# facebookresearch/omni3d

Hardware: NVIDIA H100
Metric: images/sec DLA34 Cube R-CNN train step (higher is better)
Workload: dtype bf16

## Files before the change

omni3d_b200/csrc/c3d_common.cu:

```cuda
#include <stdarg.h>
#include <string.h>
#include "c3d_common.cuh"

namespace c3d {
static thread_local char g_err[512] = "";
char* last_error_buf() { return g_err; }
int32_t set_error(int32_t code, const char* fmt, ...) {
  va_list ap; va_start(ap, fmt);
  vsnprintf(g_err, sizeof(g_err), fmt, ap);
  va_end(ap);
  return code;
}
}

extern "C" const char* c3d_last_error(void) { return c3d::last_error_buf(); }
extern "C" int32_t c3d_abi_version(void) { return 2; }
```

omni3d_b200/csrc/roi_align.cu:

```cuda
#include <cuda_bf16.h>
#include <stdlib.h>
#include "c3d_common.cuh"

namespace c3d {
using bf16 = __nv_bfloat16;

struct RoiLevels {
  const bf16* feat[5];
  float* grad[5];
  int H[5], W[5];
  float scale[5];
  int num_levels;
  int num_images;
};

struct Tap { int y0, y1, x0, x1; float w1, w2, w3, w4; bool valid; };

__device__ __forceinline__ Tap make_tap(float y, float x, int H, int W) {
  Tap t;
  t.valid = !(y < -1.0f || y > (float)H || x < -1.0f || x > (float)W);
  if (y <= 0.f) y = 0.f;
  if (x <= 0.f) x = 0.f;
  int yl = (int)y, xl = (int)x, yh, xh;
  if (yl >= H - 1) { yh = yl = H - 1; y = (float)yl; } else yh = yl + 1;
  if (xl >= W - 1) { xh = xl = W - 1; x = (float)xl; } else xh = xl + 1;
  float ly = y - yl, lx = x - xl, hy = 1.f - ly, hx = 1.f - lx;
  t.y0 = yl; t.y1 = yh; t.x0 = xl; t.x1 = xh;
  t.w1 = hy * hx; t.w2 = hy * lx; t.w3 = ly * hx; t.w4 = ly * lx;
  return t;
}

__device__ __forceinline__ void acc8(float (&a)[8], const bf16* p, float w) {
  uint4 u = __ldg(reinterpret_cast<const uint4*>(p));
  const __nv_bfloat162* h = reinterpret_cast<const __nv_bfloat162*>(&u);
#pragma unroll
  for (int i = 0; i < 4; ++i) { float2 f = __bfloat1622float2(h[i]); a[2 * i] += w * f.x; a[2 * i + 1] += w * f.y; }
}

__device__ __forceinline__ bool roi_sane(const float* roi, const RoiLevels& L) {
  const float fb = roi[0], fl = roi[1];
  return fb >= 0.f && (L.num_images <= 0 || fb < (float)L.num_images) && fl >= 0.f && fl < (float)L.num_levels &&
         isfinite(roi[2]) && isfinite(roi[3]) && isfinite(roi[4]) && isfinite(roi[5]);
}

__global__ void roi_align_kernel(RoiLevels L, const float* __restrict__ rois, int R, int C, int PH, int PW,
                                 bf16* __restrict__ out) {
  const int warps_per_block = blockDim.x >> 5;
  const int lane = threadIdx.x & 31;
  const long long nbins = (long long)R * PH * PW;
  for (long long bin = (long long)blockIdx.x * warps_per_block + (threadIdx.x >> 5); bin < nbins;
       bin += (long long)gridDim.x * warps_per_block) {
    const int pw = (int)(bin % PW), ph = (int)((bin / PW) % PH), r = (int)(bin / ((long long)PW * PH));
    const float* roi = rois + (size_t)r * 6;
    if (!roi_sane(roi, L)) {
      for (int c = lane * 8; c < C; c += 256) *reinterpret_cast<uint4*>(out + (size_t)bin * C + c) = make_uint4(0, 0, 0, 0);
      continue;
    }
    const int b = (int)roi[0], lvl = (int)roi[1];
    const float sc = L.scale[lvl];
    const int H = L.H[lvl], W = L.W[lvl];
    const float sw = roi[2] * sc - 0.5f, sh = roi[3] * sc - 0.5f;
    const float rw = roi[4] * sc - 0.5f - sw, rh = roi[5] * sc - 0.5f - sh;
    const float bh = rh / PH, bw = rw / PW;
    const int gh = (int)ceilf(rh / PH), gw = (int)ceilf(rw / PW);
    const float cnt = fmaxf((float)(gh * gw), 1.f);
    const bf16* base = L.feat[lvl] + (size_t)b * H * W * C;
    for (int c = lane * 8; c < C; c += 256) {
      float a[8];
#pragma unroll
      for (int k = 0; k < 8; ++k) a[k] = 0.f;
      for (int iy = 0; iy < gh; ++iy) {
        const float y = sh + ph * bh + (iy + 0.5f) * bh / (float)gh;
        for (int ix = 0; ix < gw; ++ix) {
          const float x = sw + pw * bw + (ix + 0.5f) * bw / (float)gw;
          Tap t = make_tap(y, x, H, W);
          if (!t.valid) continue;
          acc8(a, base + ((size_t)t.y0 * W + t.x0) * C + c, t.w1); acc8(a, base + ((size_t)t.y0 * W + t.x1) * C + c, t.w2);
          acc8(a, base + ((size_t)t.y1 * W + t.x0) * C + c, t.w3); acc8(a, base + ((size_t)t.y1 * W + t.x1) * C + c, t.w4);
        }
      }
      uint4 u;
      __nv_bfloat162* h = reinterpret_cast<__nv_bfloat162*>(&u);
#pragma unroll
      for (int i = 0; i < 4; ++i) h[i] = __floats2bfloat162_rn(a[2 * i] / cnt, a[2 * i + 1] / cnt);
      *reinterpret_cast<uint4*>(out + (size_t)bin * C + c) = u;
    }
  }
}

constexpr int kTile = 8, kTileC = 256, kListCap = 2048;
constexpr int kBwdSmem = kTile * kTile * kTileC * 4;

__global__ void __launch_bounds__(kTileC)
roi_align_bwd_kernel(RoiLevels L, const float* __restrict__ rois, int R, int C, int PH, int PW, const bf16* __restrict__ dout) {
  extern __shared__ float sacc[];
  __shared__ int slist[kListCap];
  __shared__ int s_wc[kTileC / 32];
  __shared__ int s_n, s_touch;
  const int tid = threadIdx.x, lane = tid & 31, wid = tid >> 5;
  const int b = blockIdx.y;
  int lvl = 0, band = blockIdx.x;
  while (lvl < L.num_levels - 1 && band >= (L.H[lvl] + kTile - 1) / kTile) { band -= (L.H[lvl] + kTile - 1) / kTile; ++lvl; }
  const int H = L.H[lvl], W = L.W[lvl];
  if (band * kTile >= H) return;
  const float sc = L.scale[lvl];
  const int ty0 = band * kTile, ty1 = min(H, ty0 + kTile) - 1;
  float* gmap = L.grad[lvl] + (size_t)b * H * W * C;
  for (int r0 = 0; r0 < R;) {
    if (tid == 0) s_n = 0;
    __syncthreads();
    int r = r0;
    while (r < R) {
      const int idx = r + tid;
      bool pred = false;
      if (idx < R) {
        const float* roi = rois + (size_t)idx * 6;
        if (roi_sane(roi, L) && (int)roi[0] == b && (int)roi[1] == lvl) {
          const float sh = roi[3] * sc - 0.5f, eh = roi[5] * sc - 0.5f;
          pred = (int)floorf(sh) - 1 <= ty1 && (int)floorf(eh) + 1 >= ty0;
        }
      }
      const unsigned bal = __ballot_sync(0xffffffffu, pred);
      if (lane == 0) s_wc[wid] = __popc(bal);
      __syncthreads();
      int before = 0, total = 0;
      for (int w = 0; w < kTileC / 32; ++w) { total += s_wc[w]; if (w < wid) before += s_wc[w]; }
      const int n0 = s_n;
      const bool fits = n0 + total <= kListCap;
      if (fits && pred) slist[n0 + before + __popc(bal & ((1u << lane) - 1u))] = idx;
      __syncthreads();
      if (!fits) break;
      if (tid == 0) s_n = n0 + total;
      __syncthreads();
      r += kTileC;
    }
    r0 = r;
    const int n = s_n;
    for (int tx0 = 0; tx0 < W; tx0 += kTile) {
      const int tx1 = min(W, tx0 + kTile) - 1;
      for (int cc = 0; cc < C; cc += kTileC) {
        const int c = cc + tid;
        const bool cin = c < C;
        for (int p = 0; p < kTile * kTile; ++p) sacc[p * kTileC + tid] = 0.f;
        if (tid == 0) s_touch = 0;
        __syncthreads();
        for (int li = 0; li < n; ++li) {
          const int ri = slist[li];
          const float* roi = rois + (size_t)ri * 6;
          const float sw = roi[2] * sc - 0.5f, sh = roi[3] * sc - 0.5f;
          const float rw = roi[4] * sc - 0.5f - sw, rh = roi[5] * sc - 0.5f - sh;
          if ((int)floorf(sw) - 1 > tx1 || (int)floorf(sw + rw) + 1 < tx0) continue;
          const float bh = rh / PH, bw = rw / PW;
          const int gh = (int)ceilf(rh / PH), gw = (int)ceilf(rw / PW);
          const float cnt = fmaxf((float)(gh * gw), 1.f);
          for (int ph = 0; ph < PH; ++ph) {
            if ((int)floorf(sh + ph * bh) - 1 > ty1 || (int)floorf(sh + (ph + 1) * bh) + 1 < ty0) continue;
            for (int pw = 0; pw < PW; ++pw) {
              if ((int)floorf(sw + pw * bw) - 1 > tx1 || (int)floorf(sw + (pw + 1) * bw) + 1 < tx0) continue;
              const float g = cin ? __bfloat162float(dout[(((size_t)ri * PH + ph) * PW + pw) * C + c]) / cnt : 0.f;
              for (int iy = 0; iy < gh; ++iy) {
                const float y = sh + ph * bh + (iy + 0.5f) * bh / (float)gh;
                for (int ix = 0; ix < gw; ++ix) {
                  const float x = sw + pw * bw + (ix + 0.5f) * bw / (float)gw;
                  const Tap t = make_tap(y, x, H, W);
                  if (!t.valid) continue;
                  const int ys[4] = {t.y0, t.y0, t.y1, t.y1}, xs[4] = {t.x0, t.x1, t.x0, t.x1};
                  const float ws[4] = {t.w1, t.w2, t.w3, t.w4};
#pragma unroll
                  for (int j = 0; j < 4; ++j)
                    if (ys[j] >= ty0 && ys[j] <= ty1 && xs[j] >= tx0 && xs[j] <= tx1) {
                      sacc[((ys[j] - ty0) * kTile + (xs[j] - tx0)) * kTileC + tid] += ws[j] * g;
                      if (tid == 0) s_touch = 1;
                    }
                }
              }
            }
          }
        }
        __syncthreads();
        if (s_touch && cin) {
          for (int p = 0; p < kTile * kTile; ++p) {
            const int py = ty0 + p / kTile, px = tx0 + p % kTile;
            if (py <= ty1 && px <= tx1) gmap[((size_t)py * W + px) * C + c] += sacc[p * kTileC + tid];
          }
        }
        __syncthreads();
      }
    }
  }
}

static int32_t run(bool bwd, const c3d_roi_levels* lv, const float* rois, int R, int C, int PH, int PW, void* out,
                   const void* dout, cudaStream_t st) {
  if (!lv || lv->num_levels < 1 || lv->num_levels > 5 || C % 8 != 0) return set_error(C3D_EINVAL, "roi_align: bad args");
  if (R == 0) return C3D_OK;
  RoiLevels L;
  L.num_levels = lv->num_levels;
  L.num_images = lv->num_images;
  for (int i = 0; i < 5; ++i) {
    L.feat[i] = (const bf16*)lv->feat[i]; L.grad[i] = (float*)lv->grad[i];
    L.H[i] = lv->H[i]; L.W[i] = lv->W[i]; L.scale[i] = lv->scale[i];
  }
  if (!bwd) {
    long long nbins = (long long)R * PH * PW;
    long long blocks = (nbins + 7) / 8;
    if (blocks > kNumSMs * 16) blocks = kNumSMs * 16;
    roi_align_kernel<<<(unsigned)blocks, 256, 0, st>>>(L, rois, R, C, PH, PW, (bf16*)out);
    return check_launch("roi_align");
  }
  if (L.num_images <= 0) return set_error(C3D_EINVAL, "roi_align bwd: num_images must be set");
  static bool attr = false;
  if (!attr) {
    cudaError_t e = cudaFuncSetAttribute(roi_align_bwd_kernel, cudaFuncAttributeMaxDynamicSharedMemorySize, kBwdSmem);
    if (e != cudaSuccess) return set_error(C3D_ECUDA, "roi_align bwd smem attr: %s", cudaGetErrorString(e));
    attr = true;
  }
  int bands = 0;
  for (int i = 0; i < L.num_levels; ++i) bands += (L.H[i] + kTile - 1) / kTile;
  roi_align_bwd_kernel<<<dim3((unsigned)bands, (unsigned)L.num_images), kTileC, kBwdSmem, st>>>(L, rois, R, C, PH, PW, (const bf16*)dout);
  return check_launch("roi_align bwd");
}
}

extern "C" int32_t c3d_roi_align_fwd(const c3d_roi_levels* levels, const float* rois, int32_t R, int32_t C,
                                     int32_t pooled_h, int32_t pooled_w, void* out, void* stream) {
  if (!rois && R > 0) return c3d::set_error(C3D_EINVAL, "roi_align: null rois");
  return c3d::run(false, levels, rois, R, C, pooled_h, pooled_w, out, nullptr, (cudaStream_t)stream);
}
extern "C" int32_t c3d_roi_align_bwd(const c3d_roi_levels* levels, const float* rois, int32_t R, int32_t C,
                                     int32_t pooled_h, int32_t pooled_w, const void* dout, void* stream) {
  if (!rois && R > 0) return c3d::set_error(C3D_EINVAL, "roi_align: null rois");
  return c3d::run(true, levels, rois, R, C, pooled_h, pooled_w, nullptr, dout, (cudaStream_t)stream);
}
```

omni3d_b200/kernels.py:

```python
import ctypes

import torch

from . import _lib
from ._lib import ptr, stream

vp, i32, f32 = ctypes.c_void_p, ctypes.c_int32, ctypes.c_float


def bn_finalize(stats, count, eps, momentum, running_mean, running_var):
    L = _lib.lib()
    rows, _, C = stats.shape
    mean = torch.empty(C, device=stats.device, dtype=torch.float32)
    rstd = torch.empty(C, device=stats.device, dtype=torch.float32)
    scratch = torch.empty(128 * 2 * C + 64, device=stats.device, dtype=torch.float64)
    _lib.check(L.c3d_bn_finalize(ptr(stats), rows, C, float(count), eps, momentum, ptr(running_mean), ptr(running_var),
                                 ptr(mean), ptr(rstd), ptr(scratch), stream()), launches=1)
    return mean, rstd


def bn_apply(y, mean, rstd, gamma, beta, residual=None, relu=True, out=None):
    L = _lib.lib()
    C = y.shape[-1]
    P = y.numel() // C
# ... 85 lines not shown

def preprocess_images(images, mean, std, size_divisibility=64, cpad=16):
    L = _lib.lib()
    Hm = max(im.shape[1] for im in images)
    Wm = max(im.shape[2] for im in images)
    d = size_divisibility
    Hp, Wp = (Hm + d - 1) // d * d, (Wm + d - 1) // d * d
    out = torch.empty((len(images), Hp, Wp, cpad), device=images[0].device, dtype=torch.bfloat16)
    m = (f32 * 3)(*[float(v) for v in mean])
    s = (f32 * 3)(*[float(v) for v in std])
    for im in images:
        assert im.dtype in (torch.float32, torch.uint8) and im.is_contiguous() and im.is_cuda

    def run(ims, dst):
        n = len(ims)
        ptrs = (vp * n)(*[im.data_ptr() for im in ims])
        hs = (i32 * n)(*[im.shape[1] for im in ims])
        ws = (i32 * n)(*[im.shape[2] for im in ims])
        _lib.check(L.c3d_preprocess_batch(ptrs, hs, ws, n, int(ims[0].dtype == torch.uint8), ptr(dst), Hp, Wp, cpad, m, s,
                                          stream()), launches=(n + 63) // 64)
    if all(im.dtype == images[0].dtype for im in images):
        run(images, out)
    else:
        for i, im in enumerate(images):
            run([im], out[i])
    return out


def _levels(feats, strides, grads=None):
    lv = _lib.RoiLevels()
    lv.num_levels = len(feats)
    lv.num_images = feats[0].shape[0]
    for i, f in enumerate(feats):
        lv.feat[i] = f.data_ptr()
        lv.grad[i] = grads[i].data_ptr() if grads is not None else None
        lv.H[i], lv.W[i] = f.shape[1], f.shape[2]
        lv.scale[i] = 1.0 / strides[i]
    return lv


def roi_align_fwd(feats, strides, rois, pooled=7):
    L = _lib.lib()
    C = feats[0].shape[-1]
    R = rois.shape[0]
    out = torch.empty((R, pooled, pooled, C), device=feats[0].device, dtype=torch.bfloat16)
    lv = _levels(feats, strides)
    _lib.check(L.c3d_roi_align_fwd(ctypes.byref(lv), ptr(rois), R, C, pooled, pooled, ptr(out), stream()))
    return out


def roi_align_bwd(feats, strides, rois, dout, pooled=7):
    L = _lib.lib()
    C = feats[0].shape[-1]
    grads = [torch.zeros(f.shape, device=f.device, dtype=torch.float32) for f in feats]
    lv = _levels(feats, strides, grads)
    _lib.check(L.c3d_roi_align_bwd(ctypes.byref(lv), ptr(rois), rois.shape[0], C, pooled, pooled, ptr(dout), stream()))
    return grads


def grad_finite(flat_grad, flag):
    L = _lib.lib()
    _lib.check(L.c3d_grad_finite(ptr(flat_grad), flat_grad.numel(), ptr(flag), stream()))


def sgd_momentum(p, g, mom, lr, momentum, weight_decay, grad_scale=1.0, skip_flag=None):
    L = _lib.lib()
    if torch.is_tensor(lr):
        _lib.check(L.c3d_sgd_momentum_dev(ptr(p), ptr(g), ptr(mom), p.numel(), ptr(lr), momentum, weight_decay, grad_scale,
                                          ptr(skip_flag), stream()))
    else:
        _lib.check(L.c3d_sgd_momentum(ptr(p), ptr(g), ptr(mom), p.numel(), lr, momentum, weight_decay, grad_scale,
                                      ptr(skip_flag), stream()))


_nms_ws = {}


def nms_batched(boxes, nvalid, iou_thresh, max_keep, cats=None, maxc=None, trick_max_numel=20000, ncat=0, max_per_cat=0):
    L = _lib.lib()
    B, n, _ = boxes.shape
    boxes = boxes.contiguous()
    need = L.c3d_nms_workspace_bytes(B, n)
    key = boxes.device.index
    ws = _nms_ws.get(key)
    if ws is None or ws.numel() < need:
        ws = torch.empty(need, dtype=torch.uint8, device=boxes.device)
        _nms_ws[key] = ws
    keep = torch.empty((B, max_keep), dtype=torch.int32, device=boxes.device)
    cnt = torch.empty((B,), dtype=torch.int32, device=boxes.device)
    if ncat > 0 and cats is not None:
        _lib.check(L.c3d_nms_batched_grouped(ptr(boxes), ptr(nvalid), ptr(cats), ptr(maxc), trick_max_numel, B, n, iou_thresh,
                                             max_keep, ncat, max_per_cat, ptr(keep), ptr(cnt), ptr(ws), ws.numel(), stream()),
                   launches=4)
        return keep, cnt
    _lib.check(L.c3d_nms_batched(ptr(boxes), ptr(nvalid), ptr(cats), ptr(maxc), trick_max_numel, B, n, iou_thresh,
                                 max_keep, ptr(keep), ptr(cnt), ptr(ws), ws.numel(), stream()), launches=2)
    return keep, cnt


def anchor_match(anchors, gt_boxes, gt_valid, gt_ign, fg_thresh):
    L = _lib.lib()
    A = anchors.shape[0]
    B, G, _ = gt_boxes.shape
    dev = anchors.device
    anchors, gt_boxes = anchors.contiguous().float(), gt_boxes.contiguous().float()
    v8, i8 = gt_valid.to(torch.uint8).contiguous(), gt_ign.to(torch.uint8).contiguous()
    idx = torch.empty((B, A), dtype=torch.int64, device=dev)
# ... 266 lines not shown
```

omni3d_b200/nnfunc.py:

```python
import weakref

import torch

from . import _lib
from . import conv as K
from . import kernels as Kx

_pack_cache = {}
_lin_cache = {}
_epoch = 0


def invalidate_packed():
    global _epoch
    _epoch += 1
    _pack_cache.clear()
    _lin_cache.clear()


def _cache_key(w):
    if not isinstance(w, torch.nn.Parameter):
        return None, None
    return id(w), (w.data_ptr(), w._version, _epoch, tuple(w.shape), tuple(w.stride()))

# ... 348 lines not shown
            return fn(None)
        dwb = wgrad(wb, lambda g: K.linear_wgrad(x, dzb, dw=g, chw=chw))
        dwc = wgrad(wc, lambda g: K.linear_wgrad_blocks(x, dzc, B, Fc, S, dw=g, chw=chw))
        return dx, dwb, gbb if rb else None, dwc, gbc if rc else None, None, None, None, None


class MaxPool2(torch.autograd.Function):
    @staticmethod
    def forward(ctx, x):
        ctx.sink = _sink_of(x)
        x = x.contiguous()
        ctx.save_for_backward(x)
        return Kx.maxpool2_fwd(x)

    @staticmethod
    def backward(ctx, dy):
        (x,) = ctx.saved_tensors
        sink = ctx.sink
        if sink is not None and sink.buf is not None and sink.buf.dtype == x.dtype:
            Kx.maxpool2_bwd(x, dy, into=sink.buf)
            return None
        return _deliver(sink, Kx.maxpool2_bwd(x, dy))


class MaxPool3s2(torch.autograd.Function):

    @staticmethod
    def forward(ctx, x):
        x = x.contiguous()
        ctx.save_for_backward(x)
        return Kx.maxpool3s2_fwd(x)

    @staticmethod
    def backward(ctx, dy):
        (x,) = ctx.saved_tensors
        return Kx.maxpool3s2_bwd(x, dy)


class ROIAlign(torch.autograd.Function):

    @staticmethod
    def forward(ctx, rois, strides, pooled, *feats):
        ctx.sinks = [_sink_of(f) for f in feats]
        feats = [f.contiguous() for f in feats]
        ctx.save_for_backward(rois, *feats)
        ctx.cfg = (strides, pooled)
        return Kx.roi_align_fwd(feats, strides, rois, pooled)

    @staticmethod
    def backward(ctx, dout):
        rois, *feats = ctx.saved_tensors
        strides, pooled = ctx.cfg
        grads = Kx.roi_align_bwd(feats, strides, rois, dout.contiguous(), pooled)
        return (None, None, None) + tuple(_deliver(s, g.to(torch.bfloat16)) for s, g in zip(ctx.sinks, grads))


class CubeLossRows(torch.autograd.Function):

    @staticmethod
    def forward(ctx, raw, aux):
        raw, aux = raw.contiguous().float(), aux.contiguous().float()
        ctx.save_for_backward(raw, aux)
        out = Kx.cube_loss_fwd(raw, aux)
        ctx.mark_non_differentiable()
        return out

    @staticmethod
    def backward(ctx, dout):
        raw, aux = ctx.saved_tensors
        return Kx.cube_loss_bwd(raw, aux, dout[:, :6].contiguous().float()), None


class RPNLossSums(torch.autograd.Function):

    @staticmethod
    def forward(ctx, logits, deltas, labels, matched_idx, gt_boxes, anchors, weights):
        logits, deltas = logits.contiguous().float(), deltas.contiguous().float()
        labels, matched_idx = labels.to(torch.int8).contiguous(), matched_idx.contiguous()
        gt_boxes, anchors = gt_boxes.contiguous().float(), anchors.contiguous().float()
        ctx.save_for_backward(logits, deltas, labels, matched_idx, gt_boxes, anchors)
        ctx.weights = tuple(weights)
        return Kx.rpn_loss_fwd(logits, deltas, labels, matched_idx, gt_boxes, anchors, weights)

    @staticmethod
    def backward(ctx, dacc):
        logits, deltas, labels, matched_idx, gt_boxes, anchors = ctx.saved_tensors
        dacc = dacc.contiguous().float()
        dl, dd = Kx.rpn_loss_bwd(logits, deltas, labels, matched_idx, gt_boxes, anchors, ctx.weights, dacc[0:1], dacc[1:2])
        return dl, dd, None, None, None, None, None


class BoxLoss(torch.autograd.Function):

    @staticmethod
    def forward(ctx, pred, classes, valid, boxes, gt_boxes, K, weights):
        pred = pred.contiguous().float()
        classes, valid = classes.contiguous().to(torch.int64), valid.contiguous().to(torch.uint8)
        boxes, gt_boxes = boxes.contiguous().float(), gt_boxes.contiguous().float()
        acc = Kx.box_loss_fwd(pred, classes, valid, boxes, gt_boxes, K, weights)
        ctx.save_for_backward(pred, classes, valid, boxes, gt_boxes, acc)
        ctx.cfg = (K, tuple(weights))
        nv, nfg = acc[2].clamp(min=1.0), acc[3].clamp(min=1.0)
        den = torch.stack([nv, nv, nv, nfg, nfg])
        return torch.cat([torch.cat([acc[0:2], acc[4:7]]) / den, acc[2:4]])

    @staticmethod
    def backward(ctx, g):
# ... 29 lines not shown
```

Baseline: 360.8.

## Restructure ROIAlign backward into per-tile blocks with pre-bucketed ROI lists and bf16 output

ROIAlign backward gets a small pre-pass kernel that buckets ROIs by (image, level) into a compact list. The main backward kernel then launches one block per 8x8 spatial tile instead of one per row band, and each block filters only its segment's ROIs. Each thread now handles two channels with float2 smem accumulators at half the thread count. The kernel writes bf16 gradients directly, removing the fp32 zero-fill, the read-modify-write accumulation and the separate fp32-to-bf16 cast. The cost is an extra launch plus async malloc/free per call, and tile-level ROI rescanning may duplicate filtering work.

Result: faster. 394.9 (median of 6 runs) (+9.4%).

```diff
diff --git a/omni3d_b200/csrc/c3d_common.cu b/omni3d_b200/csrc/c3d_common.cu
--- a/omni3d_b200/csrc/c3d_common.cu
+++ b/omni3d_b200/csrc/c3d_common.cu
@@ -14,4 +14,4 @@
 }
 
 extern "C" const char* c3d_last_error(void) { return c3d::last_error_buf(); }
-extern "C" int32_t c3d_abi_version(void) { return 2; }
+extern "C" int32_t c3d_abi_version(void) { return 3; }
diff --git a/omni3d_b200/csrc/roi_align.cu b/omni3d_b200/csrc/roi_align.cu
--- a/omni3d_b200/csrc/roi_align.cu
+++ b/omni3d_b200/csrc/roi_align.cu
@@ -7,7 +7,7 @@
 
 struct RoiLevels {
   const bf16* feat[5];
-  float* grad[5];
+  void* grad[5];
   int H[5], W[5];
   float scale[5];
   int num_levels;
@@ -88,120 +88,218 @@
   }
 }
 
-constexpr int kTile = 8, kTileC = 256, kListCap = 2048;
+constexpr int kTile = 8, kTileC = 256, kBwdThreads = kTileC / 2, kListCap = 2048;
 constexpr int kBwdSmem = kTile * kTile * kTileC * 4;
 
-__global__ void __launch_bounds__(kTileC)
-roi_align_bwd_kernel(RoiLevels L, const float* __restrict__ rois, int R, int C, int PH, int PW, const bf16* __restrict__ dout) {
-  extern __shared__ float sacc[];
+struct BwdScratch {
+  int* seg_off;
+  int* seg_n;
+  int* list;
+};
+
+__device__ __forceinline__ int roi_key(const float* roi, const RoiLevels& L) {
+  return roi_sane(roi, L) ? (int)roi[0] * L.num_levels + (int)roi[1] : -1;
+}
+
+__global__ void __launch_bounds__(256) roi_bwd_list_kernel(RoiLevels L, const float* __restrict__ rois, int R, BwdScratch S) {
+  __shared__ int s_wc[8];
+  const int seg = blockIdx.x, tid = threadIdx.x, lane = tid & 31, wid = tid >> 5;
+  int below = 0, n = 0;
+  for (int r0 = 0; r0 < R; r0 += 256) {
+    const int k = r0 + tid < R ? roi_key(rois + (size_t)(r0 + tid) * 6, L) : -1;
+    below += __syncthreads_count(k >= 0 && k < seg);
+    n += __syncthreads_count(k == seg);
+  }
+  int* list = S.list + below;
+  int pos = 0;
+  for (int r0 = 0; r0 < R && pos < n; r0 += 256) {
+    const bool pred = r0 + tid < R && roi_key(rois + (size_t)(r0 + tid) * 6, L) == seg;
+    const unsigned bal = __ballot_sync(0xffffffffu, pred);
+    if (lane == 0) s_wc[wid] = __popc(bal);
+    __syncthreads();
+    int before = 0, total = 0;
+    for (int w = 0; w < 8; ++w) { total += s_wc[w]; if (w < wid) before += s_wc[w]; }
+    if (pred) list[pos + before + __popc(bal & ((1u << lane) - 1u))] = r0 + tid;
+    pos += total;
+    __syncthreads();
+  }
+  if (tid == 0) { S.seg_off[seg] = below; S.seg_n[seg] = n; }
+}
+
+__device__ __forceinline__ void axis_tap(float v, int n, int& lo, int& hi, float& l) {
+  if (v <= 0.f) v = 0.f;
+  lo = (int)v;
+  if (lo >= n - 1) { hi = lo = n - 1; v = (float)lo; } else hi = lo + 1;
+  l = v - lo;
+}
+
+__global__ void __launch_bounds__(kBwdThreads, 3)
+roi_bwd_kernel(RoiLevels L, const float* __restrict__ rois, int R, int C, int PH, int PW, const bf16* __restrict__ dout,
+               BwdScratch S) {
+  extern __shared__ float2 sacc[];
   __shared__ int slist[kListCap];
-  __shared__ int s_wc[kTileC / 32];
-  __shared__ int s_n, s_touch;
+  __shared__ int s_wc[kBwdThreads / 32];
   const int tid = threadIdx.x, lane = tid & 31, wid = tid >> 5;
-  const int b = blockIdx.y;
-  int lvl = 0, band = blockIdx.x;
-  while (lvl < L.num_levels - 1 && band >= (L.H[lvl] + kTile - 1) / kTile) { band -= (L.H[lvl] + kTile - 1) / kTile; ++lvl; }
-  const int H = L.H[lvl], W = L.W[lvl];
-  if (band * kTile >= H) return;
+  int u = blockIdx.x, lvl = 0, per_image = 0;
+  for (int l = 0; l < L.num_levels; ++l) per_image += ((L.H[l] + kTile - 1) / kTile) * ((L.W[l] + kTile - 1) / kTile);
+  const int b = u / per_image;
+  u -= b * per_image;
+  while (u >= ((L.H[lvl] + kTile - 1) / kTile) * ((L.W[lvl] + kTile - 1) / kTile)) {
+    u -= ((L.H[lvl] + kTile - 1) / kTile) * ((L.W[lvl] + kTile - 1) / kTile);
+    ++lvl;
+  }
+  const int H = L.H[lvl], W = L.W[lvl], tiles_x = (W + kTile - 1) / kTile;
+  const int ty0 = (u / tiles_x) * kTile, tx0 = (u % tiles_x) * kTile;
+  const int ty1 = min(H, ty0 + kTile) - 1, tx1 = min(W, tx0 + kTile) - 1;
   const float sc = L.scale[lvl];
-  const int ty0 = band * kTile, ty1 = min(H, ty0 + kTile) - 1;
-  float* gmap = L.grad[lvl] + (size_t)b * H * W * C;
-  for (int r0 = 0; r0 < R;) {
-    if (tid == 0) s_n = 0;
-    __syncthreads();
-    int r = r0;
-    while (r < R) {
-      const int idx = r + tid;
-      bool pred = false;
-      if (idx < R) {
-        const float* roi = rois + (size_t)idx * 6;
-        if (roi_sane(roi, L) && (int)roi[0] == b && (int)roi[1] == lvl) {
-          const float sh = roi[3] * sc - 0.5f, eh = roi[5] * sc - 0.5f;
-          pred = (int)floorf(sh) - 1 <= ty1 && (int)floorf(eh) + 1 >= ty0;
+  const int seg = b * L.num_levels + lvl;
+  const int n = R > 0 ? S.seg_n[seg] : 0;
+  const int* seg_list = R > 0 ? S.list + S.seg_off[seg] : nullptr;
+  bf16* gmap = reinterpret_cast<bf16*>(L.grad[lvl]) + (size_t)b * H * W * C;
+  for (int cc = 0; cc < C; cc += kTileC) {
+    const int c = cc + 2 * tid;
+    const bool cin = c < C;
+    for (int p = 0; p < kTile * kTile; ++p) sacc[p * kBwdThreads + tid] = make_float2(0.f, 0.f);
+    for (int i0 = 0; i0 < n;) {
+      int m = 0, i = i0;
+      while (i < n) {
+        bool pred = false;
+        int ri = 0;
+        if (i + tid < n) {
+          ri = seg_list[i + tid];
+          const float* roi = rois + (size_t)ri * 6;
+          const float sw = roi[2] * sc - 0.5f, sh = roi[3] * sc - 0.5f, eh = roi[5] * sc - 0.5f;
+          const float rw = roi[4] * sc - 0.5f - sw;
+          pred = (int)floorf(sh) - 1 <= ty1 && (int)floorf(eh) + 1 >= ty0 &&
+                 !((int)floorf(sw) - 1 > tx1 || (int)floorf(sw + rw) + 1 < tx0);
         }
+        const unsigned bal = __ballot_sync(0xffffffffu, pred);
+        if (lane == 0) s_wc[wid] = __popc(bal);
+        __syncthreads();
+        int before = 0, total = 0;
+        for (int w = 0; w < kBwdThreads / 32; ++w) { total += s_wc[w]; if (w < wid) before += s_wc[w]; }
+        const bool fits = m + total <= kListCap;
+        if (fits && pred) slist[m + before + __popc(bal & ((1u << lane) - 1u))] = ri;
+        __syncthreads();
+        if (!fits) break;
+        m += total;
+        i += kBwdThreads;
       }
-      const unsigned bal = __ballot_sync(0xffffffffu, pred);
-      if (lane == 0) s_wc[wid] = __popc(bal);
-      __syncthreads();
-      int before = 0, total = 0;
-      for (int w = 0; w < kTileC / 32; ++w) { total += s_wc[w]; if (w < wid) before += s_wc[w]; }
-      const int n0 = s_n;
-      const bool fits = n0 + total <= kListCap;
-      if (fits && pred) slist[n0 + before + __popc(bal & ((1u << lane) - 1u))] = idx;
-      __syncthreads();
-      if (!fits) break;
-      if (tid == 0) s_n = n0 + total;
-      __syncthreads();
-      r += kTileC;
-    }
-    r0 = r;
-    const int n = s_n;
-    for (int tx0 = 0; tx0 < W; tx0 += kTile) {
-      const int tx1 = min(W, tx0 + kTile) - 1;
-      for (int cc = 0; cc < C; cc += kTileC) {
-        const int c = cc + tid;
-        const bool cin = c < C;
-        for (int p = 0; p < kTile * kTile; ++p) sacc[p * kTileC + tid] = 0.f;
-        if (tid == 0) s_touch = 0;
-        __syncthreads();
-        for (int li = 0; li < n; ++li) {
-          const int ri = slist[li];
-          const float* roi = rois + (size_t)ri * 6;
-          const float sw = roi[2] * sc - 0.5f, sh = roi[3] * sc - 0.5f;
-          const float rw = roi[4] * sc - 0.5f - sw, rh = roi[5] * sc - 0.5f - sh;
-          if ((int)floorf(sw) - 1 > tx1 || (int)floorf(sw + rw) + 1 < tx0) continue;
-          const float bh = rh / PH, bw = rw / PW;
-          const int gh = (int)ceilf(rh / PH), gw = (int)ceilf(rw / PW);
-          const float cnt = fmaxf((float)(gh * gw), 1.f);
-          for (int ph = 0; ph < PH; ++ph) {
-            if ((int)floorf(sh + ph * bh) - 1 > ty1 || (int)floorf(sh + (ph + 1) * bh) + 1 < ty0) continue;
-            for (int pw = 0; pw < PW; ++pw) {
-              if ((int)floorf(sw + pw * bw) - 1 > tx1 || (int)floorf(sw + (pw + 1) * bw) + 1 < tx0) continue;
-              const float g = cin ? __bfloat162float(dout[(((size_t)ri * PH + ph) * PW + pw) * C + c]) / cnt : 0.f;
-              for (int iy = 0; iy < gh; ++iy) {
-                const float y = sh + ph * bh + (iy + 0.5f) * bh / (float)gh;
-                for (int ix = 0; ix < gw; ++ix) {
-                  const float x = sw + pw * bw + (ix + 0.5f) * bw / (float)gw;
-                  const Tap t = make_tap(y, x, H, W);
-                  if (!t.valid) continue;
-                  const int ys[4] = {t.y0, t.y0, t.y1, t.y1}, xs[4] = {t.x0, t.x1, t.x0, t.x1};
-                  const float ws[4] = {t.w1, t.w2, t.w3, t.w4};
+      i0 = i;
+      for (int li = 0; li < m; ++li) {
+        const int ri = slist[li];
+        const float* roi = rois + (size_t)ri * 6;
+        const float sw = roi[2] * sc - 0.5f, sh = roi[3] * sc - 0.5f;
+        const float rw = roi[4] * sc - 0.5f - sw, rh = roi[5] * sc - 0.5f - sh;
+        const float bh = rh / PH, bw = rw / PW;
+        const int gh = (int)ceilf(rh / PH), gw = (int)ceilf(rw / PW);
+        const float cnt = fmaxf((float)(gh * gw), 1.f);
+        const bf16* dr = dout + (size_t)ri * PH * PW * C + c;
+        for (int ph = 0; ph < PH; ++ph) {
+          if ((int)floorf(sh + ph * bh) - 1 > ty1 || (int)floorf(sh + (ph + 1) * bh) + 1 < ty0) continue;
+          for (int pw = 0; pw < PW; ++pw) {
+            if ((int)floorf(sw + pw * bw) - 1 > tx1 || (int)floorf(sw + (pw + 1) * bw) + 1 < tx0) continue;
+            float2 g = make_float2(0.f, 0.f);
+            if (cin) {
+              g = __bfloat1622float2(*reinterpret_cast<const __nv_bfloat162*>(dr + (size_t)(ph * PW + pw) * C));
+              g.x = g.x / cnt; g.y = g.y / cnt;
+            }
+            for (int iy = 0; iy < gh; ++iy) {
+              const float y = sh + ph * bh + (iy + 0.5f) * bh / (float)gh;
+              if (y < -1.0f || y > (float)H) continue;
+              int y0, y1; float ly;
+              axis_tap(y, H, y0, y1, ly);
+              if (y1 < ty0 || y0 > ty1) continue;
+              const float hy = 1.f - ly;
+              for (int ix = 0; ix < gw; ++ix) {
+                const float x = sw + pw * bw + (ix + 0.5f) * bw / (float)gw;
+                if (x < -1.0f || x > (float)W) continue;
+                int x0, x1; float lx;
+                axis_tap(x, W, x0, x1, lx);
+                if (x1 < tx0 || x0 > tx1) continue;
+                const float hx = 1.f - lx;
+                const int ys[4] = {y0, y0, y1, y1}, xs[4] = {x0, x1, x0, x1};
+                const float ws[4] = {hy * hx, hy * lx, ly * hx, ly * lx};
 #pragma unroll
-                  for (int j = 0; j < 4; ++j)
-                    if (ys[j] >= ty0 && ys[j] <= ty1 && xs[j] >= tx0 && xs[j] <= tx1) {
-                      sacc[((ys[j] - ty0) * kTile + (xs[j] - tx0)) * kTileC + tid] += ws[j] * g;
-                      if (tid == 0) s_touch = 1;
-                    }
-                }
+                for (int j = 0; j < 4; ++j)
+                  if (ys[j] >= ty0 && ys[j] <= ty1 && xs[j] >= tx0 && xs[j] <= tx1) {
+                    float2* a = sacc + ((ys[j] - ty0) * kTile + (xs[j] - tx0)) * kBwdThreads + tid;
+                    float2 v = *a;
+                    v.x += ws[j] * g.x; v.y += ws[j] * g.y;
+                    *a = v;
+                  }
               }
             }
           }
         }
-        __syncthreads();
-        if (s_touch && cin) {
-          for (int p = 0; p < kTile * kTile; ++p) {
-            const int py = ty0 + p / kTile, px = tx0 + p % kTile;
-            if (py <= ty1 && px <= tx1) gmap[((size_t)py * W + px) * C + c] += sacc[p * kTileC + tid];
-          }
+      }
+      __syncthreads();
+    }
+    if (cin) {
+      for (int p = 0; p < kTile * kTile; ++p) {
+        const int y = ty0 + p / kTile, x = tx0 + p % kTile;
+        if (y <= ty1 && x <= tx1) {
+          const float2 v = sacc[p * kBwdThreads + tid];
+          *reinterpret_cast<__nv_bfloat162*>(gmap + ((size_t)y * W + x) * C + c) =
+              __floats2bfloat162_rn(0.f + v.x, 0.f + v.y);
         }
-        __syncthreads();
       }
     }
   }
+}
+
+static size_t align16(size_t n) { return (n + 15) & ~(size_t)15; }
+
+static int32_t run_bwd(const RoiLevels& L, const float* rois, int R, int C, int PH, int PW, const bf16* dout, cudaStream_t st) {
+  static bool attr = false;
+  if (!attr) {
+    cudaError_t e = cudaFuncSetAttribute(roi_bwd_kernel, cudaFuncAttributeMaxDynamicSharedMemorySize, kBwdSmem);
+    if (e != cudaSuccess) return set_error(C3D_ECUDA, "roi_align bwd smem attr: %s", cudaGetErrorString(e));
+    attr = true;
+  }
+  long long units = 0;
+  for (int i = 0; i < L.num_levels; ++i)
+    units += (long long)((L.H[i] + kTile - 1) / kTile) * ((L.W[i] + kTile - 1) / kTile);
+  units *= L.num_images;
+  if (units == 0) return C3D_OK;
+  if (units > 0x7fffffffLL) return set_error(C3D_EINVAL, "roi_align bwd: maps too large");
+  const int nseg = L.num_images * L.num_levels;
+  BwdScratch S{};
+  void* scratch = nullptr;
+  if (R > 0) {
+    const size_t seg_bytes = align16((size_t)nseg * 4);
+    cudaError_t e = cudaMallocAsync(&scratch, 2 * seg_bytes + (size_t)R * 4, st);
+    if (e != cudaSuccess) return set_error(C3D_ECUDA, "roi_align bwd scratch: %s", cudaGetErrorString(e));
+    char* p = static_cast<char*>(scratch);
+    S.seg_off = reinterpret_cast<int*>(p);
+    S.seg_n = reinterpret_cast<int*>(p + seg_bytes);
+    S.list = reinterpret_cast<int*>(p + 2 * seg_bytes);
+    roi_bwd_list_kernel<<<(unsigned)nseg, 256, 0, st>>>(L, rois, R, S);
+    int32_t rc = check_launch("roi_bwd_list_kernel");
+    if (rc != C3D_OK) { cudaFreeAsync(scratch, st); return rc; }
+  }
+  roi_bwd_kernel<<<(unsigned)units, kBwdThreads, kBwdSmem, st>>>(L, rois, R, C, PH, PW, dout, S);
+  int32_t rc = check_launch("roi_bwd_kernel");
+  if (scratch) {
+    cudaError_t e = cudaFreeAsync(scratch, st);
+    if (rc == C3D_OK && e != cudaSuccess) rc = set_error(C3D_ECUDA, "roi_align bwd scratch free: %s", cudaGetErrorString(e));
+  }
+  return rc;
 }
 
 static int32_t run(bool bwd, const c3d_roi_levels* lv, const float* rois, int R, int C, int PH, int PW, void* out,
                    const void* dout, cudaStream_t st) {
   if (!lv || lv->num_levels < 1 || lv->num_levels > 5 || C % 8 != 0) return set_error(C3D_EINVAL, "roi_align: bad args");
-  if (R == 0) return C3D_OK;
+  if (R < 0 || PH < 1 || PW < 1) return set_error(C3D_EINVAL, "roi_align: bad sizes");
   RoiLevels L;
   L.num_levels = lv->num_levels;
   L.num_images = lv->num_images;
   for (int i = 0; i < 5; ++i) {
-    L.feat[i] = (const bf16*)lv->feat[i]; L.grad[i] = (float*)lv->grad[i];
+    L.feat[i] = (const bf16*)lv->feat[i]; L.grad[i] = lv->grad[i];
     L.H[i] = lv->H[i]; L.W[i] = lv->W[i]; L.scale[i] = lv->scale[i];
   }
   if (!bwd) {
+    if (R == 0) return C3D_OK;
     long long nbins = (long long)R * PH * PW;
     long long blocks = (nbins + 7) / 8;
     if (blocks > kNumSMs * 16) blocks = kNumSMs * 16;
@@ -209,16 +307,9 @@
     return check_launch("roi_align");
   }
   if (L.num_images <= 0) return set_error(C3D_EINVAL, "roi_align bwd: num_images must be set");
-  static bool attr = false;
-  if (!attr) {
-    cudaError_t e = cudaFuncSetAttribute(roi_align_bwd_kernel, cudaFuncAttributeMaxDynamicSharedMemorySize, kBwdSmem);
-    if (e != cudaSuccess) return set_error(C3D_ECUDA, "roi_align bwd smem attr: %s", cudaGetErrorString(e));
-    attr = true;
-  }
-  int bands = 0;
-  for (int i = 0; i < L.num_levels; ++i) bands += (L.H[i] + kTile - 1) / kTile;
-  roi_align_bwd_kernel<<<dim3((unsigned)bands, (unsigned)L.num_images), kTileC, kBwdSmem, st>>>(L, rois, R, C, PH, PW, (const bf16*)dout);
-  return check_launch("roi_align bwd");
+  for (int i = 0; i < L.num_levels; ++i)
+    if (!L.grad[i] || L.H[i] < 1 || L.W[i] < 1) return set_error(C3D_EINVAL, "roi_align bwd: level %d needs a map", i);
+  return run_bwd(L, rois, R, C, PH, PW, (const bf16*)dout, st);
 }
 }
 
diff --git a/omni3d_b200/kernels.py b/omni3d_b200/kernels.py
--- a/omni3d_b200/kernels.py
+++ b/omni3d_b200/kernels.py
@@ -161,7 +161,7 @@
 def roi_align_bwd(feats, strides, rois, dout, pooled=7):
     L = _lib.lib()
     C = feats[0].shape[-1]
-    grads = [torch.zeros(f.shape, device=f.device, dtype=torch.float32) for f in feats]
+    grads = [torch.empty(f.shape, device=f.device, dtype=torch.bfloat16) for f in feats]
     lv = _levels(feats, strides, grads)
     _lib.check(L.c3d_roi_align_bwd(ctypes.byref(lv), ptr(rois), rois.shape[0], C, pooled, pooled, ptr(dout), stream()))
     return grads
diff --git a/omni3d_b200/nnfunc.py b/omni3d_b200/nnfunc.py
--- a/omni3d_b200/nnfunc.py
+++ b/omni3d_b200/nnfunc.py
@@ -424,7 +424,7 @@
         rois, *feats = ctx.saved_tensors
         strides, pooled = ctx.cfg
         grads = Kx.roi_align_bwd(feats, strides, rois, dout.contiguous(), pooled)
-        return (None, None, None) + tuple(_deliver(s, g.to(torch.bfloat16)) for s, g in zip(ctx.sinks, grads))
+        return (None, None, None) + tuple(_deliver(s, g) for s, g in zip(ctx.sinks, grads))
 
 
 class CubeLossRows(torch.autograd.Function):
```

## Bucket ROIs per image/level and rework RoIAlign backward into work-list scatter

Applied to the files above, without the earlier changes.

Adds a single-block bucketing kernel that sorts ROIs by (image, level) into offset/index lists. The backward tile kernel then reads only its own bucket instead of rescanning and filtering all ROIs in every band block. It also builds per-tile lists of active bins and samples, which spreads the per-sample tap work across all threads, and writes every tile in place of read-modify-write. That lets the Python side drop the zero-fill of the gradient buffers. The cost is a second launch, an async allocation on every call, a larger shared-memory footprint, and more barrier-heavy inner loops.

Result: faster. 392.6 before, 420.5 after, median of 6 (+7.1%).

```diff
diff --git a/omni3d_b200/csrc/c3d_common.cu b/omni3d_b200/csrc/c3d_common.cu
--- a/omni3d_b200/csrc/c3d_common.cu
+++ b/omni3d_b200/csrc/c3d_common.cu
@@ -14,4 +14,4 @@
 }
 
 extern "C" const char* c3d_last_error(void) { return c3d::last_error_buf(); }
-extern "C" int32_t c3d_abi_version(void) { return 2; }
+extern "C" int32_t c3d_abi_version(void) { return 3; }
diff --git a/omni3d_b200/csrc/roi_align.cu b/omni3d_b200/csrc/roi_align.cu
--- a/omni3d_b200/csrc/roi_align.cu
+++ b/omni3d_b200/csrc/roi_align.cu
@@ -14,6 +14,26 @@
   int num_images;
 };
 
+struct RoiGeom { float sw, sh, rw, rh, bw, bh, cnt; int gw, gh; };
+
+__device__ __forceinline__ RoiGeom roi_geom(const float* roi, float sc, int PH, int PW) {
+  RoiGeom g;
+  g.sw = fmaf(roi[2], sc, -0.5f);
+  g.sh = fmaf(roi[3], sc, -0.5f);
+  g.rw = __fsub_rn(fmaf(roi[4], sc, -0.5f), g.sw);
+  g.rh = __fsub_rn(fmaf(roi[5], sc, -0.5f), g.sh);
+  g.bw = __fdiv_rn(g.rw, (float)PW);
+  g.bh = __fdiv_rn(g.rh, (float)PH);
+  g.gw = (int)ceilf(g.bw);
+  g.gh = (int)ceilf(g.bh);
+  g.cnt = fmaxf((float)(g.gh * g.gw), 1.f);
+  return g;
+}
+
+__device__ __forceinline__ float sample_at(float s, int p, float b, int i, int n) {
+  return __fadd_rn(fmaf((float)p, b, s), __fdiv_rn(__fmul_rn(__fadd_rn((float)i, 0.5f), b), (float)n));
+}
+
 struct Tap { int y0, y1, x0, x1; float w1, w2, w3, w4; bool valid; };
 
 __device__ __forceinline__ Tap make_tap(float y, float x, int H, int W) {
@@ -24,9 +44,9 @@
   int yl = (int)y, xl = (int)x, yh, xh;
   if (yl >= H - 1) { yh = yl = H - 1; y = (float)yl; } else yh = yl + 1;
   if (xl >= W - 1) { xh = xl = W - 1; x = (float)xl; } else xh = xl + 1;
-  float ly = y - yl, lx = x - xl, hy = 1.f - ly, hx = 1.f - lx;
+  const float ly = __fsub_rn(y, (float)yl), lx = __fsub_rn(x, (float)xl), hy = __fsub_rn(1.f, ly), hx = __fsub_rn(1.f, lx);
   t.y0 = yl; t.y1 = yh; t.x0 = xl; t.x1 = xh;
-  t.w1 = hy * hx; t.w2 = hy * lx; t.w3 = ly * hx; t.w4 = ly * lx;
+  t.w1 = __fmul_rn(hy, hx); t.w2 = __fmul_rn(hy, lx); t.w3 = __fmul_rn(ly, hx); t.w4 = __fmul_rn(ly, lx);
   return t;
 }
 
@@ -57,22 +77,18 @@
       continue;
     }
     const int b = (int)roi[0], lvl = (int)roi[1];
-    const float sc = L.scale[lvl];
     const int H = L.H[lvl], W = L.W[lvl];
-    const float sw = roi[2] * sc - 0.5f, sh = roi[3] * sc - 0.5f;
-    const float rw = roi[4] * sc - 0.5f - sw, rh = roi[5] * sc - 0.5f - sh;
-    const float bh = rh / PH, bw = rw / PW;
-    const int gh = (int)ceilf(rh / PH), gw = (int)ceilf(rw / PW);
-    const float cnt = fmaxf((float)(gh * gw), 1.f);
+    const RoiGeom g = roi_geom(roi, L.scale[lvl], PH, PW);
+    const float cnt = g.cnt;
     const bf16* base = L.feat[lvl] + (size_t)b * H * W * C;
     for (int c = lane * 8; c < C; c += 256) {
       float a[8];
 #pragma unroll
       for (int k = 0; k < 8; ++k) a[k] = 0.f;
-      for (int iy = 0; iy < gh; ++iy) {
-        const float y = sh + ph * bh + (iy + 0.5f) * bh / (float)gh;
-        for (int ix = 0; ix < gw; ++ix) {
-          const float x = sw + pw * bw + (ix + 0.5f) * bw / (float)gw;
+      for (int iy = 0; iy < g.gh; ++iy) {
+        const float y = sample_at(g.sh, ph, g.bh, iy, g.gh);
+        for (int ix = 0; ix < g.gw; ++ix) {
+          const float x = sample_at(g.sw, pw, g.bw, ix, g.gw);
           Tap t = make_tap(y, x, H, W);
           if (!t.valid) continue;
           acc8(a, base + ((size_t)t.y0 * W + t.x0) * C + c, t.w1); acc8(a, base + ((size_t)t.y0 * W + t.x1) * C + c, t.w2);
@@ -88,16 +104,122 @@
   }
 }
 
-constexpr int kTile = 8, kTileC = 256, kListCap = 2048;
-constexpr int kBwdSmem = kTile * kTile * kTileC * 4;
-
-__global__ void __launch_bounds__(kTileC)
-roi_align_bwd_kernel(RoiLevels L, const float* __restrict__ rois, int R, int C, int PH, int PW, const bf16* __restrict__ dout) {
-  extern __shared__ float sacc[];
-  __shared__ int slist[kListCap];
-  __shared__ int s_wc[kTileC / 32];
-  __shared__ int s_n, s_touch;
+constexpr int kTile = 8, kTileC = 256, kSlots = 32, kEntCap = 4 * kTileC;
+constexpr int kBucketThreads = 1024, kBucketWarps = kBucketThreads / 32;
+
+struct BwdSmem {
+  float acc[kTile * kTile][kTileC];
+  float g[kSlots][kTileC];
+  int2 ent[kEntCap];
+  int roi[kTileC];
+  int rect[kTileC];
+  int bins[kTileC + 1];
+  float sh[kSlots], sw[kSlots], bh[kSlots], bw[kSlots], cnt[kSlots];
+  int gh[kSlots], gw[kSlots], ph[kSlots], pw[kSlots], ri[kSlots], iy[kSlots], ix[kSlots], nix[kSlots];
+  int items[kSlots + 1];
+  int warp[kTileC / 32];
+};
+
+__device__ __forceinline__ int warp_inclusive_scan(int x, int lane) {
+#pragma unroll
+  for (int o = 1; o < 32; o <<= 1) {
+    const int y = __shfl_up_sync(0xffffffffu, x, o);
+    if (lane >= o) x += y;
+  }
+  return x;
+}
+
+__device__ __forceinline__ int block_exclusive_scan(int v, int* s_warp, int& total) {
+  const int lane = threadIdx.x & 31, wid = threadIdx.x >> 5;
+  const int x = warp_inclusive_scan(v, lane);
+  if (lane == 31) s_warp[wid] = x;
+  __syncthreads();
+  int before = 0;
+  total = 0;
+#pragma unroll
+  for (int w = 0; w < kTileC / 32; ++w) {
+    const int t = s_warp[w];
+    if (w < wid) before += t;
+    total += t;
+  }
+  return before + x - v;
+}
+
+__device__ __forceinline__ int roi_bucket(const float* roi, const RoiLevels& L) {
+  return roi_sane(roi, L) ? (int)roi[0] * L.num_levels + (int)roi[1] : -1;
+}
+
+__global__ void __launch_bounds__(kBucketThreads)
+roi_bucket_kernel(RoiLevels L, const float* __restrict__ rois, int R, int nb, int* __restrict__ wk, int* __restrict__ off,
+                  int* __restrict__ idx) {
+  __shared__ int s_part[kBucketWarps];
+  __shared__ int s_carry;
   const int tid = threadIdx.x, lane = tid & 31, wid = tid >> 5;
+  for (int i = tid; i < kBucketWarps * nb; i += kBucketThreads) wk[i] = 0;
+  if (tid == 0) s_carry = 0;
+  __syncthreads();
+  const int per = (R + kBucketWarps - 1) / kBucketWarps;
+  const int lo = min(R, wid * per), hi = min(R, lo + per);
+  int* mine = wk + (size_t)wid * nb;
+  for (int r0 = lo; r0 < hi; r0 += 32) {
+    const int r = r0 + lane;
+    const int k = r < hi ? roi_bucket(rois + (size_t)r * 6, L) : -1;
+    const unsigned peers = __match_any_sync(0xffffffffu, k);
+    if (k >= 0 && lane == __ffs(peers) - 1) atomicAdd(&mine[k], __popc(peers));
+  }
+  __syncthreads();
+  for (int k0 = 0; k0 < nb; k0 += kBucketThreads) {
+    const int k = k0 + tid;
+    int tot = 0;
+    if (k < nb)
+      for (int w = 0; w < kBucketWarps; ++w) tot += wk[(size_t)w * nb + k];
+    const int x = warp_inclusive_scan(tot, lane);
+    if (lane == 31) s_part[wid] = x;
+    __syncthreads();
+    int run = s_carry + x - tot, chunk = 0;
+    for (int w = 0; w < kBucketWarps; ++w) {
+      if (w < wid) run += s_part[w];
+      chunk += s_part[w];
+    }
+    if (k < nb) {
+      off[k] = run;
+      for (int w = 0; w < kBucketWarps; ++w) {
+        const int c = wk[(size_t)w * nb + k];
+        wk[(size_t)w * nb + k] = run;
+        run += c;
+      }
+    }
+    __syncthreads();
+    if (tid == 0) s_carry += chunk;
+    __syncthreads();
+  }
+  if (tid == 0) off[nb] = s_carry;
+  for (int r0 = lo; r0 < hi; r0 += 32) {
+    const int r = r0 + lane;
+    const int k = r < hi ? roi_bucket(rois + (size_t)r * 6, L) : -1;
+    const unsigned peers = __match_any_sync(0xffffffffu, k);
+    const int leader = __ffs(peers) - 1;
+    int base = 0;
+    if (k >= 0 && lane == leader) base = atomicAdd(&mine[k], __popc(peers));
+    base = __shfl_sync(0xffffffffu, base, leader);
+    if (k >= 0) idx[base + __popc(peers & ((1u << lane) - 1u))] = r;
+  }
+}
+
+__device__ __forceinline__ void sample_range(float s, float st, int n, int t0, int t1, int& first, int& count) {
+  const float slop = 2.f + 1e-5f * fabsf(s) / st;
+  const float lo = ceilf(((float)t0 - 1.f - s) / st - 0.5f - slop), hi = floorf(((float)t1 + 1.f - s) / st - 0.5f + slop);
+  first = (int)fmaxf(lo, 0.f);
+  const int last = (int)fminf(hi, (float)(n - 1));
+  count = max(0, last - first + 1);
+}
+
+__global__ void __launch_bounds__(kTileC, 2)
+roi_align_bwd_kernel(RoiLevels L, const float* __restrict__ rois, const int* __restrict__ off, const int* __restrict__ idx,
+                     int C, int PH, int PW, const bf16* __restrict__ dout) {
+  extern __shared__ __align__(16) unsigned char smem_raw[];
+  BwdSmem& S = *reinterpret_cast<BwdSmem*>(smem_raw);
+  const int tid = threadIdx.x, lane = tid & 31;
   const int b = blockIdx.y;
   int lvl = 0, band = blockIdx.x;
   while (lvl < L.num_levels - 1 && band >= (L.H[lvl] + kTile - 1) / kTile) { band -= (L.H[lvl] + kTile - 1) / kTile; ++lvl; }
@@ -105,86 +227,121 @@
   if (band * kTile >= H) return;
   const float sc = L.scale[lvl];
   const int ty0 = band * kTile, ty1 = min(H, ty0 + kTile) - 1;
+  const int key = b * L.num_levels + lvl;
+  const int* list = idx + off[key];
+  const int n = off[key + 1] - off[key];
   float* gmap = L.grad[lvl] + (size_t)b * H * W * C;
-  for (int r0 = 0; r0 < R;) {
-    if (tid == 0) s_n = 0;
-    __syncthreads();
-    int r = r0;
-    while (r < R) {
-      const int idx = r + tid;
-      bool pred = false;
-      if (idx < R) {
-        const float* roi = rois + (size_t)idx * 6;
-        if (roi_sane(roi, L) && (int)roi[0] == b && (int)roi[1] == lvl) {
-          const float sh = roi[3] * sc - 0.5f, eh = roi[5] * sc - 0.5f;
-          pred = (int)floorf(sh) - 1 <= ty1 && (int)floorf(eh) + 1 >= ty0;
-        }
-      }
-      const unsigned bal = __ballot_sync(0xffffffffu, pred);
-      if (lane == 0) s_wc[wid] = __popc(bal);
-      __syncthreads();
-      int before = 0, total = 0;
-      for (int w = 0; w < kTileC / 32; ++w) { total += s_wc[w]; if (w < wid) before += s_wc[w]; }
-      const int n0 = s_n;
-      const bool fits = n0 + total <= kListCap;
-      if (fits && pred) slist[n0 + before + __popc(bal & ((1u << lane) - 1u))] = idx;
-      __syncthreads();
-      if (!fits) break;
-      if (tid == 0) s_n = n0 + total;
-      __syncthreads();
-      r += kTileC;
-    }
-    r0 = r;
-    const int n = s_n;
-    for (int tx0 = 0; tx0 < W; tx0 += kTile) {
-      const int tx1 = min(W, tx0 + kTile) - 1;
-      for (int cc = 0; cc < C; cc += kTileC) {
-        const int c = cc + tid;
-        const bool cin = c < C;
-        for (int p = 0; p < kTile * kTile; ++p) sacc[p * kTileC + tid] = 0.f;
-        if (tid == 0) s_touch = 0;
-        __syncthreads();
-        for (int li = 0; li < n; ++li) {
-          const int ri = slist[li];
-          const float* roi = rois + (size_t)ri * 6;
-          const float sw = roi[2] * sc - 0.5f, sh = roi[3] * sc - 0.5f;
-          const float rw = roi[4] * sc - 0.5f - sw, rh = roi[5] * sc - 0.5f - sh;
-          if ((int)floorf(sw) - 1 > tx1 || (int)floorf(sw + rw) + 1 < tx0) continue;
-          const float bh = rh / PH, bw = rw / PW;
-          const int gh = (int)ceilf(rh / PH), gw = (int)ceilf(rw / PW);
-          const float cnt = fmaxf((float)(gh * gw), 1.f);
-          for (int ph = 0; ph < PH; ++ph) {
-            if ((int)floorf(sh + ph * bh) - 1 > ty1 || (int)floorf(sh + (ph + 1) * bh) + 1 < ty0) continue;
-            for (int pw = 0; pw < PW; ++pw) {
-              if ((int)floorf(sw + pw * bw) - 1 > tx1 || (int)floorf(sw + (pw + 1) * bw) + 1 < tx0) continue;
-              const float g = cin ? __bfloat162float(dout[(((size_t)ri * PH + ph) * PW + pw) * C + c]) / cnt : 0.f;
-              for (int iy = 0; iy < gh; ++iy) {
-                const float y = sh + ph * bh + (iy + 0.5f) * bh / (float)gh;
-                for (int ix = 0; ix < gw; ++ix) {
-                  const float x = sw + pw * bw + (ix + 0.5f) * bw / (float)gw;
-                  const Tap t = make_tap(y, x, H, W);
-                  if (!t.valid) continue;
-                  const int ys[4] = {t.y0, t.y0, t.y1, t.y1}, xs[4] = {t.x0, t.x1, t.x0, t.x1};
-                  const float ws[4] = {t.w1, t.w2, t.w3, t.w4};
-#pragma unroll
-                  for (int j = 0; j < 4; ++j)
-                    if (ys[j] >= ty0 && ys[j] <= ty1 && xs[j] >= tx0 && xs[j] <= tx1) {
-                      sacc[((ys[j] - ty0) * kTile + (xs[j] - tx0)) * kTileC + tid] += ws[j] * g;
-                      if (tid == 0) s_touch = 1;
-                    }
-                }
+  for (int tx0 = 0; tx0 < W; tx0 += kTile) {
+    const int tx1 = min(W, tx0 + kTile) - 1;
+    for (int cc = 0; cc < C; cc += kTileC) {
+      const int c = cc + tid;
+#pragma unroll 8
+      for (int p = 0; p < kTile * kTile; ++p) S.acc[p][tid] = 0.f;
+      for (int w0 = 0; w0 < n; w0 += kTileC) {
+        int nbin = 0, rect = 0, ri = 0;
+        if (w0 + tid < n) {
+          ri = list[w0 + tid];
+          const RoiGeom g = roi_geom(rois + (size_t)ri * 6, sc, PH, PW);
+          if (g.gh > 0 && g.gw > 0) {
+            int ph0 = PH, ph1 = -1, pw0 = PW, pw1 = -1;
+            for (int ph = 0; ph < PH; ++ph)
+              if ((int)floorf(g.sh + ph * g.bh) - 1 <= ty1 && (int)floorf(g.sh + (ph + 1) * g.bh) + 1 >= ty0) {
+                ph0 = min(ph0, ph);
+                ph1 = ph;
               }
+            for (int pw = 0; pw < PW; ++pw)
+              if ((int)floorf(g.sw + pw * g.bw) - 1 <= tx1 && (int)floorf(g.sw + (pw + 1) * g.bw) + 1 >= tx0) {
+                pw0 = min(pw0, pw);
+                pw1 = pw;
+              }
+            if (ph1 >= ph0 && pw1 >= pw0) {
+              nbin = (ph1 - ph0 + 1) * (pw1 - pw0 + 1);
+              rect = ph0 | pw0 << 8 | (pw1 - pw0 + 1) << 16;
             }
           }
         }
+        int nbins;
+        const int first = block_exclusive_scan(nbin, S.warp, nbins);
+        S.roi[tid] = ri;
+        S.rect[tid] = rect;
+        S.bins[tid] = first;
+        if (tid == 0) S.bins[kTileC] = nbins;
         __syncthreads();
-        if (s_touch && cin) {
-          for (int p = 0; p < kTile * kTile; ++p) {
-            const int py = ty0 + p / kTile, px = tx0 + p % kTile;
-            if (py <= ty1 && px <= tx1) gmap[((size_t)py * W + px) * C + c] += sacc[p * kTileC + tid];
+        for (int s0 = 0; s0 < nbins; s0 += kSlots) {
+          const int ns = min(kSlots, nbins - s0);
+          if (tid < 32) {
+            int items = 0;
+            if (lane < ns) {
+              const int bin = s0 + lane;
+              int lo = 0, hi = kTileC;
+              while (hi - lo > 1) {
+                const int mid = (lo + hi) >> 1;
+                if (S.bins[mid] <= bin) lo = mid; else hi = mid;
+              }
+              const int rc = S.rect[lo], r = S.roi[lo], local = bin - S.bins[lo], npw = rc >> 16;
+              const int ph = (rc & 255) + local / npw, pw = ((rc >> 8) & 255) + local % npw;
+              const RoiGeom g = roi_geom(rois + (size_t)r * 6, sc, PH, PW);
+              int iy0, niy, ix0, nix;
+              sample_range(fmaf((float)ph, g.bh, g.sh), __fdiv_rn(g.bh, (float)g.gh), g.gh, ty0, ty1, iy0, niy);
+              sample_range(fmaf((float)pw, g.bw, g.sw), __fdiv_rn(g.bw, (float)g.gw), g.gw, tx0, tx1, ix0, nix);
+              S.sh[lane] = g.sh; S.sw[lane] = g.sw; S.bh[lane] = g.bh; S.bw[lane] = g.bw; S.cnt[lane] = g.cnt;
+              S.gh[lane] = g.gh; S.gw[lane] = g.gw; S.ph[lane] = ph; S.pw[lane] = pw; S.ri[lane] = r;
+              S.iy[lane] = iy0; S.ix[lane] = ix0; S.nix[lane] = nix;
+              items = niy * nix;
+            }
+            S.items[lane + 1] = warp_inclusive_scan(items, lane);
+            if (lane == 0) S.items[0] = 0;
           }
+          __syncthreads();
+          for (int s = 0; s < ns; ++s)
+            S.g[s][tid] = c < C ? __fdiv_rn(__bfloat162float(dout[(((size_t)S.ri[s] * PH + S.ph[s]) * PW + S.pw[s]) * C + c]), S.cnt[s])
+                                : 0.f;
+          const int nitems = S.items[ns];
+          for (int i0 = 0; i0 < nitems; i0 += kTileC) {
+            const int k = i0 + tid;
+            unsigned mask = 0;
+            int slot = 0;
+            Tap t = {};
+            if (k < nitems) {
+              int lo = 0, hi = ns;
+              while (hi - lo > 1) {
+                const int mid = (lo + hi) >> 1;
+                if (S.items[mid] <= k) lo = mid; else hi = mid;
+              }
+              slot = lo;
+              const int local = k - S.items[slot], nx = S.nix[slot];
+              const float y = sample_at(S.sh[slot], S.ph[slot], S.bh[slot], S.iy[slot] + local / nx, S.gh[slot]);
+              const float x = sample_at(S.sw[slot], S.pw[slot], S.bw[slot], S.ix[slot] + local % nx, S.gw[slot]);
+              t = make_tap(y, x, H, W);
+              if (t.valid) {
+                const bool r0 = t.y0 >= ty0 && t.y0 <= ty1, r1 = t.y1 >= ty0 && t.y1 <= ty1;
+                const bool c0 = t.x0 >= tx0 && t.x0 <= tx1, c1 = t.x1 >= tx0 && t.x1 <= tx1;
+                mask = (r0 && c0) | (r0 && c1) << 1 | (r1 && c0) << 2 | (r1 && c1) << 3;
+              }
+            }
+            int nent;
+            int q = block_exclusive_scan(__popc(mask), S.warp, nent);
+            const int tag = slot << 6;
+            if (mask & 1) S.ent[q++] = make_int2(tag | (t.y0 - ty0) * kTile + (t.x0 - tx0), __float_as_int(t.w1));
+            if (mask & 2) S.ent[q++] = make_int2(tag | (t.y0 - ty0) * kTile + (t.x1 - tx0), __float_as_int(t.w2));
+            if (mask & 4) S.ent[q++] = make_int2(tag | (t.y1 - ty0) * kTile + (t.x0 - tx0), __float_as_int(t.w3));
+            if (mask & 8) S.ent[q] = make_int2(tag | (t.y1 - ty0) * kTile + (t.x1 - tx0), __float_as_int(t.w4));
+            __syncthreads();
+            for (int e = 0; e < nent; ++e) {
+              const int2 en = S.ent[e];
+              float& a = S.acc[en.x & 63][tid];
+              a = fmaf(__int_as_float(en.y), S.g[en.x >> 6][tid], a);
+            }
+            __syncthreads();
+          }
+          __syncthreads();
         }
-        __syncthreads();
+      }
+      if (c < C) {
+        for (int p = 0; p < kTile * kTile; ++p) {
+          const int py = ty0 + p / kTile, px = tx0 + p % kTile;
+          if (py <= ty1 && px <= tx1) gmap[((size_t)py * W + px) * C + c] = S.acc[p][tid];
+        }
       }
     }
   }
@@ -193,7 +350,7 @@
 static int32_t run(bool bwd, const c3d_roi_levels* lv, const float* rois, int R, int C, int PH, int PW, void* out,
                    const void* dout, cudaStream_t st) {
   if (!lv || lv->num_levels < 1 || lv->num_levels > 5 || C % 8 != 0) return set_error(C3D_EINVAL, "roi_align: bad args");
-  if (R == 0) return C3D_OK;
+  if (R < 0) return set_error(C3D_EINVAL, "roi_align: negative R");
   RoiLevels L;
   L.num_levels = lv->num_levels;
   L.num_images = lv->num_images;
@@ -202,6 +359,7 @@
     L.H[i] = lv->H[i]; L.W[i] = lv->W[i]; L.scale[i] = lv->scale[i];
   }
   if (!bwd) {
+    if (R == 0) return C3D_OK;
     long long nbins = (long long)R * PH * PW;
     long long blocks = (nbins + 7) / 8;
     if (blocks > kNumSMs * 16) blocks = kNumSMs * 16;
@@ -209,16 +367,31 @@
     return check_launch("roi_align");
   }
   if (L.num_images <= 0) return set_error(C3D_EINVAL, "roi_align bwd: num_images must be set");
+  if (PH < 1 || PW < 1 || PH > 255 || PW > 255) return set_error(C3D_EINVAL, "roi_align bwd: pooled size outside [1, 255]");
   static bool attr = false;
   if (!attr) {
-    cudaError_t e = cudaFuncSetAttribute(roi_align_bwd_kernel, cudaFuncAttributeMaxDynamicSharedMemorySize, kBwdSmem);
+    cudaError_t e = cudaFuncSetAttribute(roi_align_bwd_kernel, cudaFuncAttributeMaxDynamicSharedMemorySize, (int)sizeof(BwdSmem));
     if (e != cudaSuccess) return set_error(C3D_ECUDA, "roi_align bwd smem attr: %s", cudaGetErrorString(e));
     attr = true;
   }
-  int bands = 0;
-  for (int i = 0; i < L.num_levels; ++i) bands += (L.H[i] + kTile - 1) / kTile;
-  roi_align_bwd_kernel<<<dim3((unsigned)bands, (unsigned)L.num_images), kTileC, kBwdSmem, st>>>(L, rois, R, C, PH, PW, (const bf16*)dout);
-  return check_launch("roi_align bwd");
+  const int nb = L.num_images * L.num_levels;
+  int* off = nullptr;
+  cudaError_t e = cudaMallocAsync(reinterpret_cast<void**>(&off), ((size_t)(kBucketWarps + 1) * nb + 1 + R) * sizeof(int), st);
+  if (e != cudaSuccess) return set_error(C3D_ECUDA, "roi_align bwd buckets: %s", cudaGetErrorString(e));
+  int* wk = off + nb + 1;
+  int* idx = wk + (size_t)kBucketWarps * nb;
+  roi_bucket_kernel<<<1, kBucketThreads, 0, st>>>(L, rois, R, nb, wk, off, idx);
+  int32_t rc = check_launch("roi_align bwd buckets");
+  if (rc == C3D_OK) {
+    int bands = 0;
+    for (int i = 0; i < L.num_levels; ++i) bands += (L.H[i] + kTile - 1) / kTile;
+    roi_align_bwd_kernel<<<dim3((unsigned)bands, (unsigned)L.num_images), kTileC, sizeof(BwdSmem), st>>>(
+        L, rois, off, idx, C, PH, PW, (const bf16*)dout);
+    rc = check_launch("roi_align bwd");
+  }
+  e = cudaFreeAsync(off, st);
+  if (rc == C3D_OK && e != cudaSuccess) rc = set_error(C3D_ECUDA, "roi_align bwd buckets free: %s", cudaGetErrorString(e));
+  return rc;
 }
 }
 
diff --git a/omni3d_b200/kernels.py b/omni3d_b200/kernels.py
--- a/omni3d_b200/kernels.py
+++ b/omni3d_b200/kernels.py
@@ -161,7 +161,7 @@
 def roi_align_bwd(feats, strides, rois, dout, pooled=7):
     L = _lib.lib()
     C = feats[0].shape[-1]
-    grads = [torch.zeros(f.shape, device=f.device, dtype=torch.float32) for f in feats]
+    grads = [torch.empty(f.shape, device=f.device, dtype=torch.float32) for f in feats]
     lv = _levels(feats, strides, grads)
     _lib.check(L.c3d_roi_align_bwd(ctypes.byref(lv), ptr(rois), rois.shape[0], C, pooled, pooled, ptr(dout), stream()))
     return grads
```
